# Amin-Nadimy/P-A_multigrids

Hardware: NVIDIA B200
Metric: DG DOF-updates/s per smoother sweep (higher is better)
Workload: dtype f64

## Files before the change

### p-a_multigrids_b200/csrc/pamg_api.cu

```cuda
#include <cuda_runtime.h>
#include <dlfcn.h>

#include <algorithm>
#include <cmath>
#include <cstdio>
#include <cstring>
#include <string>
#include <vector>

#include "pamg_internal.h"
#include "pamg_kernels.cuh"
#include "pamg_unstr.cuh"

using namespace pamg;

namespace {
typedef struct ncclComm* ncclComm_t;
typedef struct { char internal[128]; } ncclUniqueId;
enum { ncclUint8 = 1, ncclInt32 = 2, ncclFloat64 = 8, ncclSum = 0, ncclMax = 2, ncclMin = 3, ncclSuccess = 0 };
struct NcclApi {
  void* lib = nullptr;
  int (*GetUniqueId)(ncclUniqueId*) = nullptr;
  int (*CommInitRank)(ncclComm_t*, int, ncclUniqueId, int) = nullptr;
  int (*CommDestroy)(ncclComm_t) = nullptr;
// ... 433 lines not shown
  }
  if (g_nccl.GroupEnd() != ncclSuccess) return fail(h, PAMG_ERR_CUDA, "ncclGroupEnd failed in halo exchange");
  return PAMG_OK;
}

int launch_halo_kernel(pamg_handle* h, LevelDev& L, HaloMode mode, const double* src, double* ovl) {
  const bool cut = mode != HALO_DIRICHLET && !h->plan.peers.empty();
  if ((mode == HALO_CUT || mode == HALO_UNPACK) && !cut) return PAMG_OK;
  const int level = (int)(&L - h->lev.data()) + 1;
  HaloArgs a;
  a.tnew = src; a.told = L.told; a.ovl = ovl; a.ovl_old = L.ovl_old; a.xg = h->xg;
  a.dst_strip = h->dst_strip; a.rev = h->rev; a.strip_of = h->strip_of;
  a.bc_scale = (h->p.coarse_bc_zero && level + h->level_offset > 1) ? 0.0 : 1.0;
  a.U = h->U; a.s = L.s; a.with_old = (mode == HALO_ALL) ? 1 : 0; a.what = mode; a.nstrips = h->plan.nstrips;
  a.cut_lf = h->cut_lf; a.ncut = (int)h->plan.cut_lf.size();
  a.bc_kind = h->bc_kind; a.bc_val = h->bc_val;
  a.x.npeers = 0;
  if (cut && h->comm && h->p2p_enabled && !h->p2p_ready && !h->p2p_failed && !h->capturing && h->level_offset == 0) {
    int rc = p2p_setup(h);
    if (rc) return rc;
  }
  const bool fused_x = cut && h->p2p_ready;
  if (fused_x) { int rc = p2p_args(h, L, ovl, a.x); if (rc) return rc; }
  const long long n = (mode == HALO_CUT ? (long long)a.ncut : mode == HALO_UNPACK ? (long long)a.ncut * 3 : (long long)h->U * 3) * L.S;
  int grid = grid_for(h, n);
  if (fused_x) grid = std::min(grid, h->nsm * std::min(std::max(h->kc.halo, 1), 4));
  k_halo<<<grid, TPB, 0, h->stream>>>(a);
  h->launches++;
  CK(cudaGetLastError());
  if (cut && !fused_x) return exchange_halo_nccl(h, L, ovl);
  return PAMG_OK;
}

int exchange_told(pamg_handle* h, LevelDev& L) {
  int rc = launch_halo_kernel(h, L, HALO_CUT, L.told, L.ovl_old);
  if (!rc) halo_exchanged(L, HALO_CUT, false);
  return rc;
}

int launch_halo(pamg_handle* h, int level, HaloMode mode) {
  LevelDev& L = h->lev[level - 1];
  if (mode == HALO_UNPACK && !(h->p2p_ready && L.cut == CUT_STAGED)) return fail(h, PAMG_ERR_STATE, "nothing staged to unpack");
  int rc;
  if (mode == HALO_ALL && (rc = exchange_told(h, L))) return rc;
  if ((rc = launch_halo_kernel(h, L, mode, tnew_ptr(L), L.ovlb[L.ovl_cur]))) return rc;
  if (mode == HALO_UNPACK) unpacked(L);
  else halo_exchanged(L, mode, true);
  return PAMG_OK;
}

bool producer_level(const LevelDev& L) { return L.s >= 6 && L.s <= 8; }

int add_old_time_terms(pamg_handle* h);

int launch_build_rhs(pamg_handle* h) {
  LevelDev& L = h->lev[0];
  RhsArgs a;
  a.told = L.told; a.rhs = L.rhs; a.pc = L.pc; a.xg = h->xg; a.dt = h->p.dt; a.source_coef = h->p.source_coef;
  a.nelem = L.nelem; a.s = L.s; a.literal_source = h->p.literal_source;
  k_build_rhs<<<grid_for(h, L.nelem), TPB, 0, h->stream>>>(a);
  h->launches++;
  CK(cudaGetLastError());
  if (L.pc_old) { int rc = add_old_time_terms(h); if (rc) return rc; }
  L.rhs_valid = true;
  return PAMG_OK;
}

template <typename K>
int configure_one(pamg_handle* h, K kern, int threads, size_t smem, int& resident) {
  CK(cudaFuncSetAttribute(kern, cudaFuncAttributeMaxDynamicSharedMemorySize, (int)smem));
  CK(cudaOccupancyMaxActiveBlocksPerMultiprocessor(&resident, kern, threads, smem));
  if (resident < 1) resident = 1;
  return PAMG_OK;
}
template <bool FACE>
int configure_face(pamg_handle* h) {
  int rc, dummy = 0;
  const int f = FACE ? 1 : 0;
  if ((rc = configure_one(h, k_element_win2<MODE_JACOBI, FACE>, WIN2_THREADS, WIN_SMEM_BYTES, h->kc.win2[f]))) return rc;
  if ((rc = configure_one(h, k_element_win2<MODE_RESID, FACE>, WIN2_THREADS, WIN_SMEM_BYTES, dummy))) return rc;
  if ((rc = configure_one(h, k_element_win2<MODE_RICH, FACE>, WIN2_THREADS, WIN_SMEM_BYTES, dummy))) return rc;
  if (FACE) {
    if ((rc = configure_one(h, k_element_win2<MODE_JACOBI, FACE, true>, WIN2_THREADS, WIN_SMEM_BYTES, h->kc.win2x))) return rc;
    if ((rc = configure_one(h, k_element_win2<MODE_JACOBI, FACE, false, true>, WIN2_THREADS, WIN_SMEM_BYTES, dummy))) return rc;
    if ((rc = configure_one(h, k_element_win2<MODE_JACOBI, FACE, true, true>, WIN2_THREADS, WIN_SMEM_BYTES, dummy))) return rc;
    if ((rc = configure_one(h, k_element_win2<MODE_RICH, FACE, true>, WIN2_THREADS, WIN_SMEM_BYTES, dummy))) return rc;
  }
  if ((rc = configure_one(h, k_element_win<MODE_JACOBI, FACE>, TPB, WIN_SMEM_BYTES, h->kc.win[f]))) return rc;
  if ((rc = configure_one(h, k_element_win<MODE_RESID, FACE>, TPB, WIN_SMEM_BYTES, dummy))) return rc;
  if ((rc = configure_one(h, k_element_win<MODE_RICH, FACE>, TPB, WIN_SMEM_BYTES, dummy))) return rc;
  if (!FACE && (rc = configure_one(h, k_element_win<MODE_GS, false>, TPB, WIN_SMEM_BYTES, dummy))) return rc;
  if ((rc = configure_one(h, k_element_tma<MODE_JACOBI, FACE>, TPB, TMA_SMEM_BYTES, h->kc.tma[f]))) return rc;
  if ((rc = configure_one(h, k_element_tma<MODE_RESID, FACE>, TPB, TMA_SMEM_BYTES, dummy))) return rc;
  if ((rc = configure_one(h, k_element_tma<MODE_RICH, FACE>, TPB, TMA_SMEM_BYTES, dummy))) return rc;
  if ((rc = configure_one(h, k_element_tma<MODE_GS, FACE>, TPB, TMA_SMEM_BYTES, dummy))) return rc;
  return PAMG_OK;
}
int configure_kernels(pamg_handle* h) {
  if (h->kc.done) return PAMG_OK;
  int rc;
  if ((rc = configure_face<true>(h))) return rc;
  if ((rc = configure_face<false>(h))) return rc;
  if ((rc = configure_one(h, k_gs_win2<false>, WIN2_THREADS, GSW_SMEM_BYTES, h->kc.gs2))) return rc;
  if ((rc = configure_one(h, k_gs_win2<true>, WIN2_THREADS, GSW_SMEM_BYTES, h->kc.gs2x))) return rc;
  if ((rc = configure_one(h, k_gs_win, TPB, GSW_SMEM_BYTES, h->kc.gs))) return rc;
  CK(cudaOccupancyMaxActiveBlocksPerMultiprocessor(&h->kc.halo, k_halo, TPB, 0));
  if (h->kc.halo < 1) h->kc.halo = 1;
  cudaFuncAttributes fa;
  CK(cudaFuncGetAttributes(&fa, k_halo));
  CK(cudaFuncGetAttributes(&fa, k_gs_small));
  CK(cudaFuncGetAttributes(&fa, k_build_rhs));
  CK(cudaFuncGetAttributes(&fa, k_restrict));
  CK(cudaFuncGetAttributes(&fa, k_prolong_literal));
  CK(cudaFuncGetAttributes(&fa, k_prolong_p1));
  CK(cudaFuncGetAttributes(&fa, k_reduce_partials));
  CK(cudaFuncGetAttributes(&fa, k_fill));
  CK(cudaFuncGetAttributes(&fa, k_push));
  CK(cudaFuncGetAttributes(&fa, k_wait_flags));
  CK(cudaFuncGetAttributes(&fa, k_output_fields));
  CK(cudaFuncGetAttributes(&fa, k_element_direct2<MODE_JACOBI, true>));
  CK(cudaFuncGetAttributes(&fa, k_element_direct2<MODE_JACOBI, false>));
  CK(cudaFuncGetAttributes(&fa, k_element_direct2<MODE_RESID, true>));
  CK(cudaFuncGetAttributes(&fa, k_element_direct2<MODE_RESID, false>));
  CK(cudaFuncGetAttributes(&fa, k_element_direct2<MODE_RICH, true>));
  CK(cudaFuncGetAttributes(&fa, k_element_direct2<MODE_RICH, false>));
  CK(cudaFuncGetAttributes(&fa, k_element_direct2<MODE_GS, false>));
  h->kc.done = true;
  return PAMG_OK;
}

ElemArgs elem_args(const pamg_handle* h, const LevelDev& L, const double* Tin, double* Tout, int colour, bool use_strips,
                   bool write_next) {
  ElemArgs a;
  a.xsend = L.xsend; a.xsync = h->p2p_sync ? h->p2p_sync + (size_t)(&L - h->lev.data()) * P2P_WORDS : nullptr;
  a.Tin = Tin; a.Tout = Tout; a.rhs = L.rhs; a.ovl = L.ovlb[L.ovl_cur]; a.pc = L.pc; a.strip_of = h->strip_of; a.hmap = h->hmap;
  a.nsrc = (use_strips || Tin == Tout) ? nullptr : h->nsrc;
  a.ovl_next = write_next ? L.ovlb[L.ovl_cur ^ 1] : nullptr; a.dst_strip = h->dst_strip; a.rev = h->rev; a.nstrips = h->plan.nstrips;
  a.partial = h->partial; a.omega = h->p.omega; a.rsign = (double)h->p.residual_sign; a.nelem = L.nelem; a.s = L.s;
  a.colour = colour; a.partial_off = 0;
  return a;
}

struct ElemOverride { const double* ovl; const double* pc; double rsign; };

template <int MODE>
int launch_element(pamg_handle* h, LevelDev& L, const double* Tin, double* Tout, int colour, int grid, bool use_strips,
                   bool write_next = false, bool xchg = false, bool norm = false, const ElemOverride* ov = nullptr) {
  ElemArgs a = elem_args(h, L, Tin, Tout, colour, use_strips, write_next);
  if (MODE == MODE_RESID) xchg = false;
  if (ov) { a.ovl = ov->ovl; a.pc = ov->pc; a.rsign = ov->rsign; }
  const int f = h->p.face_terms ? 1 : 0;
  constexpr bool FACE_OK = MODE != MODE_GS;
  const bool prof = !ov && h->profiling && h->pev_used + 2 <= (int)h->pev.size();
  if (prof) CK(cudaEventRecord(h->pev[h->pev_used], h->stream));
  if (MODE != MODE_GS && producer_level(L)) {
    auto kern = xchg ? k_element_win2<MODE == MODE_RESID ? MODE_JACOBI : MODE, true, true>
                     : h->p.face_terms ? k_element_win2<MODE, true> : k_element_win2<MODE, false>;
    if (norm) kern = xchg ? k_element_win2<MODE == MODE_JACOBI ? MODE_JACOBI : MODE, true, true, MODE == MODE_JACOBI>
                          : k_element_win2<MODE == MODE_JACOBI ? MODE_JACOBI : MODE, true, false, MODE == MODE_JACOBI>;
    const int tgrid = (int)std::max(1ll, std::min(L.nelem / TPB, (long long)h->nsm * (xchg ? h->kc.win2x : h->kc.win2[f])));
    kern<<<tgrid, WIN2_THREADS, WIN_SMEM_BYTES, h->stream>>>(a);
    if (MODE == MODE_RESID || norm) h->last_partials = tgrid;
  } else if (L.C >= TPB && L.s <= 8) {
    auto kern = h->p.face_terms && FACE_OK ? k_element_win<MODE, FACE_OK> : k_element_win<MODE, false>;
    const int tgrid = (int)std::max(1ll, std::min(L.nelem / TPB, (long long)h->nsm * h->kc.win[f]));
    kern<<<tgrid, TPB, WIN_SMEM_BYTES, h->stream>>>(a);
    if (MODE == MODE_RESID) h->last_partials = tgrid;
  } else if (L.C >= TPB) {
    auto kern = h->p.face_terms ? k_element_tma<MODE, true> : k_element_tma<MODE, false>;
    const int tgrid = (int)std::max(1ll, std::min((L.nelem + TPB - 1) / TPB, (long long)h->nsm * h->kc.tma[f]));
    kern<<<tgrid, TPB, TMA_SMEM_BYTES, h->stream>>>(a);
    if (MODE == MODE_RESID) h->last_partials = tgrid;
  } else {
    if (MODE == MODE_RESID) h->last_partials = grid;
    if (h->p.face_terms && FACE_OK) k_element_direct2<MODE, FACE_OK><<<grid, TPB, 0, h->stream>>>(a);
    else k_element_direct2<MODE, false><<<grid, TPB, 0, h->stream>>>(a);
  }
  if (prof) { CK(cudaEventRecord(h->pev[h->pev_used + 1], h->stream)); h->pev_used += 2; }
  h->launches++;
  CK(cudaGetLastError());
  return PAMG_OK;
}

int add_old_time_terms(pamg_handle* h) {
  LevelDev& L = h->lev[0];
  int rc;
  if (h->p.face_terms && (rc = exchange_told(h, L))) return rc;
  const int grid = grid_for(h, L.nelem);
  if (2 * grid > h->npartial) return fail(h, PAMG_ERR_STATE, "partial buffer too small");
  const ElemOverride ov = {L.ovl_old, L.pc_old, -1.0};
  if ((rc = launch_element<MODE_RESID>(h, L, L.told, L.res, 0, grid, false, false, false, false, &ov))) return rc;
  CK(cudaMemcpyAsync(L.rhs, L.res, (size_t)L.ndof * sizeof(double), cudaMemcpyDeviceToDevice, h->stream));
  return PAMG_OK;
}

bool gs_small_ok(const pamg_handle* h, const LevelDev& L) { return h->p.face_terms && L.C <= TPB; }

int launch_gs_one_pass(pamg_handle* h, LevelDev& L, const double* Tin, double* Tout, bool use_strips, bool write_next, bool xchg) {
  const ElemArgs a = elem_args(h, L, Tin, Tout, 1, use_strips, write_next);
  if (gs_small_ok(h, L)) {
    const long long ppc = TPB / L.C, nparents = L.nelem / L.C;
    const int sgrid = (int)std::max(1ll, std::min((nparents + ppc - 1) / ppc, (long long)h->nsm * 8));
    k_gs_small<<<sgrid, TPB, 0, h->stream>>>(a);
    h->launches++;
    CK(cudaGetLastError());
    return PAMG_OK;
  }
  const bool producer = producer_level(L);
  const int resident = producer ? (xchg ? h->kc.gs2x : h->kc.gs2) : h->kc.gs;
  const bool prof = h->profiling && h->pev_used + 2 <= (int)h->pev.size();
  if (prof) CK(cudaEventRecord(h->pev[h->pev_used], h->stream));
  const int tgrid = (int)std::max(1ll, std::min(L.nelem / TPB, (long long)h->nsm * resident));
  if (producer && xchg) k_gs_win2<true><<<tgrid, WIN2_THREADS, GSW_SMEM_BYTES, h->stream>>>(a);
  else if (producer) k_gs_win2<false><<<tgrid, WIN2_THREADS, GSW_SMEM_BYTES, h->stream>>>(a);
  else k_gs_win<<<tgrid, TPB, GSW_SMEM_BYTES, h->stream>>>(a);
  if (prof) { CK(cudaEventRecord(h->pev[h->pev_used + 1], h->stream)); h->pev_used += 2; }
  h->launches++;
  CK(cudaGetLastError());
  return PAMG_OK;
}

bool norm_fusable(const pamg_handle* h, const LevelDev& L) { return h->p.face_terms && producer_level(L); }

int do_smooth(pamg_handle* h, int level, int solver, int nsweeps, bool norm_first = false) {
  LevelDev& L = h->lev[level - 1];
  if (level == 1 && !L.rhs_valid) { int rc = launch_build_rhs(h); if (rc) return rc; }
  const int grid = grid_for(h, L.nelem);
  if (solver < 1 || solver > 4) return fail(h, PAMG_ERR_ARG, "solver must be 1 (Jacobi), 2 (Richardson) or 3 (Gauss-Seidel)");
  for (int sw = 0; sw < nsweeps; ++sw) {
    L.tnew_alias = true;
    const bool gs = solver == 3 || solver == 4;
    const bool in_place = gs && !(h->p.face_terms && L.s <= 8);
    const bool fusedk = h->p.face_terms && producer_level(L);
    const bool use_strips = in_place || fusedk;
    const bool xs = fusedk && h->p2p_ready && L.xsend && !h->plan.peers.empty();
    int rc = ensure_strips(h, level, use_strips);
    if (rc) return rc;
    if (solver == 1 || solver == 2) {
      rc = (solver == 1) ? launch_element<MODE_JACOBI>(h, L, L.T[L.cur], L.T[L.cur ^ 1], 0, grid, use_strips, fusedk, xs,
                                                       norm_first && sw == 0)
                         : launch_element<MODE_RICH>(h, L, L.T[L.cur], L.T[L.cur ^ 1], 0, grid, use_strips, fusedk, xs);
      if (rc) return rc;
      L.cur ^= 1;
      L.tnew_alias = false;
    } else if (!in_place) {
      rc = launch_gs_one_pass(h, L, L.T[L.cur], L.T[L.cur ^ 1], use_strips, fusedk, xs);
      if (rc) return rc;
      L.cur ^= 1;
      L.tnew_alias = false;
    } else {
      if (sw == nsweeps - 1 && h->p.keep_tnew_gs) { rc = materialise_tnew(h, L); if (rc) return rc; }
      rc = launch_element<MODE_GS>(h, L, L.T[L.cur], L.T[L.cur], 0, grid, true);
      if (rc) return rc;
      rc = launch_element<MODE_GS>(h, L, L.T[L.cur], L.T[L.cur], 1, grid, true);
      if (rc) return rc;
    }
    if (fusedk) L.ovl_cur ^= 1;
    sweep_done(h, L, fusedk, xs);
  }
  return PAMG_OK;
}

int queue_norms(pamg_handle* h) {
  k_reduce_partials<<<1, 1024, 0, h->stream>>>(h->partial, h->last_partials, h->out3);
  h->launches++;
  CK(cudaGetLastError());
  if (h->comm && h->nranks > 1) {
    g_nccl.GroupStart();
    g_nccl.AllReduce(h->out3, h->out3, 1, ncclFloat64, ncclSum, h->comm, h->stream);
    g_nccl.AllReduce(h->out3 + 1, h->out3 + 1, 2, ncclFloat64, ncclMax, h->comm, h->stream);
    if (g_nccl.GroupEnd() != ncclSuccess) return fail(h, PAMG_ERR_CUDA, "ncclAllReduce failed");
  }
  CK(cudaMemcpyAsync(h->out3_host, h->out3, 3 * sizeof(double), cudaMemcpyDeviceToHost, h->stream));
  return PAMG_OK;
}

int do_residual(pamg_handle* h, int level, double* l2, double* linf, double* smax, bool queue_only = false) {
  LevelDev& L = h->lev[level - 1];
  if (level == 1 && !L.rhs_valid) { int rc = launch_build_rhs(h); if (rc) return rc; }
  const int grid = grid_for(h, L.nelem);
  if (2 * grid > h->npartial) return fail(h, PAMG_ERR_STATE, "partial buffer too small");
  const bool use_strips = L.strips_valid;
  int rc = ensure_strips(h, level, use_strips);
  if (rc) return rc;
  rc = launch_element<MODE_RESID>(h, L, tnew_ptr(L), L.res, 0, grid, use_strips);
  if (rc) return rc;
  if (l2 || linf || smax) {
    if ((rc = queue_norms(h))) return rc;
    if (queue_only || h->capturing) return PAMG_OK;
    CK(cudaStreamSynchronize(h->stream));
    if ((rc = p2p_check(h))) return rc;
    if (l2) *l2 = std::sqrt(h->out3_host[0]);
    if (linf) *linf = h->out3_host[1];
    if (smax) *smax = h->out3_host[2];
  }
  return PAMG_OK;
}

int do_restrict(pamg_handle* h, int fine_level) {
  if (fine_level >= (int)h->lev.size()) return PAMG_OK;
  LevelDev& F = h->lev[fine_level - 1];
  LevelDev& Cc = h->lev[fine_level];
  XferArgs a;
  a.src = F.res; a.dst = Cc.rhs; a.ncoarse = Cc.nelem; a.sc = Cc.s; a.mode = h->p.transfer;
  k_restrict<<<grid_for(h, Cc.nelem), TPB, 0, h->stream>>>(a);
  h->launches++;
  CK(cudaGetLastError());
  Cc.rhs_valid = true;
  return PAMG_OK;
}

int do_prolong(pamg_handle* h, int fine_level, bool keep_tnew = true) {
  if (fine_level >= (int)h->lev.size()) return fail(h, PAMG_ERR_ARG, "no coarser level to prolong from");
  LevelDev& F = h->lev[fine_level - 1];
  LevelDev& Cc = h->lev[fine_level];
  XferArgs a;
  a.ncoarse = Cc.nelem; a.sc = Cc.s; a.mode = h->p.transfer;
  if (h->p.transfer == 0) {
    int rc = materialise_tnew(h, F);
    if (rc) return rc;
    a.src = tnew_ptr(Cc); a.dst = F.T[F.cur ^ 1];
    k_prolong_literal<<<grid_for(h, Cc.nelem), TPB, 0, h->stream>>>(a);
  } else {
// ... 1504 lines not shown
```

### p-a_multigrids_b200/csrc/pamg_kernels.cuh

```cuda
#pragma once
#include <cstdint>

namespace pamg {

constexpr int NPC = 88;
constexpr int PC_FOLD = 24;
constexpr int PC_DPEN = 56;
constexpr int PC_WB = 60;
enum { PC_CM = 0, PC_K11 = 1, PC_K12, PC_K13, PC_K22, PC_K23, PC_K33, PC_ADV = 7, PC_FL = 10, PC_PENI = 13, PC_W = 16, PC_PENX = 19 };

constexpr int TPB = 256;

enum { MODE_JACOBI = 0, MODE_RESID = 1, MODE_GS = 2, MODE_RICH = 3 };

constexpr int P2P_SLOTS = 4;
constexpr int P2P_MAXP = 16;
enum { P2P_EPOCH = 0, P2P_COUNT = 1, P2P_WORDS = 8 };
struct P2PArgs {
  const double* send;
  int send_base;
  double* strips;
  uint4* remote[P2P_MAXP];
  long long rstride[P2P_MAXP];
  long long soff[P2P_MAXP + 1];
// ... 140 lines not shown
  const double* e = a.ovl + ((size_t)strip * S + p) * 3;
  va = __ldg(e + (hm & 3)); vb = __ldg(e + (hm >> 2));
}

__device__ __forceinline__ void halo_pair(const ElemArgs& a, int u, int mf, int slot0, int S, double& va, double& vb) {
  const int d = a.nsrc ? __ldg(a.nsrc + u * 3 + mf) : -1;
  ext_pair(a, d, __ldg(a.strip_of + u * 3 + mf), __ldg(a.hmap + u * 3 + mf), slot0, S, va, vb);
}

__device__ __forceinline__ void p2p_advance(unsigned long long* sync, unsigned long long e64) {
  if (atomicAdd(sync + P2P_COUNT, 1ull) == (unsigned long long)gridDim.x - 1) {
    sync[P2P_COUNT] = 0;
    *(volatile unsigned long long*)(sync + P2P_EPOCH) = e64 + 1;
  }
}

__device__ __forceinline__ void block_partial(double acc_sum, double acc_abs, double acc_max, double* partial) {
  for (int o = 16; o > 0; o >>= 1) {
    acc_sum += __shfl_xor_sync(0xffffffffu, acc_sum, o);
    acc_abs = fmax(acc_abs, __shfl_xor_sync(0xffffffffu, acc_abs, o));
    acc_max = fmax(acc_max, __shfl_xor_sync(0xffffffffu, acc_max, o));
  }
  __shared__ double sh[3][TPB / 32];
  const int w = threadIdx.x >> 5, l = threadIdx.x & 31;
  if (l == 0) { sh[0][w] = acc_sum; sh[1][w] = acc_abs; sh[2][w] = acc_max; }
  __syncthreads();
  if (threadIdx.x == 0) {
    double s0 = 0, s1 = 0, s2 = 0;
    for (int i = 0; i < TPB / 32; ++i) { s0 += sh[0][i]; s1 = fmax(s1, sh[1][i]); s2 = fmax(s2, sh[2][i]); }
    partial[(size_t)blockIdx.x * 3 + 0] = s0;
    partial[(size_t)blockIdx.x * 3 + 1] = s1;
    partial[(size_t)blockIdx.x * 3 + 2] = s2;
  }
}

__device__ __forceinline__ uint32_t smem_u32(const void* p) { return (uint32_t)__cvta_generic_to_shared(p); }
__device__ __forceinline__ void mbar_init(uint64_t* bar, int count) {
  asm volatile("mbarrier.init.shared::cta.b64 [%0], %1;" ::"r"(smem_u32(bar)), "r"(count) : "memory");
}
__device__ __forceinline__ void mbar_expect_tx(uint64_t* bar, uint32_t bytes) {
  asm volatile("mbarrier.arrive.expect_tx.shared::cta.b64 _, [%0], %1;" ::"r"(smem_u32(bar)), "r"(bytes) : "memory");
}
__device__ __forceinline__ void mbar_wait(uint64_t* bar, uint32_t parity) {
  asm volatile(
      "{\n"
      ".reg .pred p;\n"
      "LAB_WAIT_%=:\n"
      "mbarrier.try_wait.parity.shared::cta.b64 p, [%0], %1;\n"
      "@p bra LAB_DONE_%=;\n"
      "bra LAB_WAIT_%=;\n"
      "LAB_DONE_%=:\n"
      "}\n" ::"r"(smem_u32(bar)), "r"(parity) : "memory");
}
__device__ __forceinline__ void tma_load_1d(void* smem_dst, const void* gsrc, uint32_t bytes, uint64_t* bar) {
  asm volatile("cp.async.bulk.shared::cluster.global.mbarrier::complete_tx::bytes [%0], [%1], %2, [%3];" ::"r"(
                   smem_u32(smem_dst)), "l"(gsrc), "r"(bytes), "r"(smem_u32(bar)) : "memory");
}
__device__ __forceinline__ void tma_store_1d(void* gdst, const void* smem_src, uint32_t bytes) {
  asm volatile("cp.async.bulk.global.shared::cta.bulk_group [%0], [%1], %2;" ::"l"(gdst), "r"(smem_u32(smem_src)),
               "r"(bytes) : "memory");
}
__device__ __forceinline__ void tma_store_commit() { asm volatile("cp.async.bulk.commit_group;" ::: "memory"); }
__device__ __forceinline__ void tma_store_wait_read() { asm volatile("cp.async.bulk.wait_group.read 0;" ::: "memory"); }
__device__ __forceinline__ void tma_store_wait_all() { asm volatile("cp.async.bulk.wait_group 0;" ::: "memory"); }
__device__ __forceinline__ void fence_async_smem() { asm volatile("fence.proxy.async.shared::cta;" ::: "memory"); }

__host__ __device__ __forceinline__ void child_from_ele0(int k, int s, int& r, int& ipos, int& len) {
  const int b = 2 << s, S = 1 << s;
  int m = (int)(((float)b - sqrtf((float)(b * b - 4 * k))) * 0.5f);
  m = max(0, min(m, S - 1));
  m -= (m * (b - m) > k);
  m += (m + 1 < S) && ((m + 1) * (b - m - 1) <= k);
  m -= (m * (b - m) > k);
  r = m + 1;
  ipos = k - m * (b - m) + 1;
  len = b + 1 - 2 * r;
}

__host__ __device__ __forceinline__ void child_advance(int s, int b, int k_next, int& r, int& ipos) {
  if (k_next < TPB) { int len; child_from_ele0(k_next, s, r, ipos, len); return; }
  ipos += TPB;
  int len = b + 1 - 2 * r;
  while (ipos > len) { ipos -= len; len -= 2; ++r; }
}

constexpr int TMA_T_DOUBLES = 3 * TPB + 8;
constexpr int NSTAGE = 3;
constexpr size_t TMA_SMEM_BYTES = sizeof(double) * (NSTAGE * (TMA_T_DOUBLES + 3 * TPB) + 2 * 3 * TPB) + 16 * NSTAGE + 64;

struct ParentRegs {
  double cm, k11, k12, k13, k22, k23, k33, adv1, adv2, adv3, fl1, fl2, fl3, pi1, pi2, pi3;
  double w1, w2, w3;
  double px1, px2, px3;
};
static_assert(sizeof(ParentRegs) == 22 * sizeof(double), "ParentRegs must mirror the pc table");
__device__ __forceinline__ void load_parent(const double* __restrict__ pc, ParentRegs& P) {
  double* d = reinterpret_cast<double*>(&P);
#pragma unroll
  for (int i = 0; i < 22; ++i) d[i] = __ldg(pc + i);
}

struct Folded { double a11, a12, a13, a21, a22, a23, a31, a32, a33, c1, c2, c3, w1, w2, w3, pad; };
static_assert(sizeof(Folded) == 16 * sizeof(double), "Folded layout");

template <int MODE, bool WITH_R = false>
__device__ __forceinline__ void elem_apply_folded(const Folded& F, const double* ext, int mask, double T1, double T2,
                                                  double T3, const FaceIn& fi, double b1, double b2, double b3,
                                                  double rsign, double& o1, double& o2, double& o3, double* rr = nullptr) {
  double ax1 = F.a11 * T1 + F.a12 * T2 + F.a13 * T3;
  double ax2 = F.a21 * T1 + F.a22 * T2 + F.a23 * T3;
  double ax3 = F.a31 * T1 + F.a32 * T2 + F.a33 * T3;
  ax1 += F.c1 * (2.0 * fi.n1a + fi.n1b); ax3 += F.c1 * (fi.n1a + 2.0 * fi.n1b);
  ax3 += F.c2 * (2.0 * fi.n2a + fi.n2b); ax2 += F.c2 * (fi.n2a + 2.0 * fi.n2b);
  ax2 += F.c3 * (2.0 * fi.n3a + fi.n3b); ax1 += F.c3 * (fi.n3a + 2.0 * fi.n3b);
  double w1 = F.w1, w2 = F.w2, w3 = F.w3;
  if (mask) {
    if (mask & 1) { const double dp = ext[0], da = T1 - fi.n1a, db = T3 - fi.n1b; ax1 += dp * (2.0 * da + db); ax3 += dp * (da + 2.0 * db); }
    if (mask & 2) { const double dp = ext[1], da = T3 - fi.n2a, db = T2 - fi.n2b; ax3 += dp * (2.0 * da + db); ax2 += dp * (da + 2.0 * db); }
    if (mask & 4) { const double dp = ext[2], da = T2 - fi.n3a, db = T1 - fi.n3b; ax2 += dp * (2.0 * da + db); ax1 += dp * (da + 2.0 * db); }
    const double* wb = ext + 4 + mask * 3;
    w1 = wb[0]; w2 = wb[1]; w3 = wb[2];
  }
  if (WITH_R) { rr[0] = rsign * (ax1 - b1); rr[1] = rsign * (ax2 - b2); rr[2] = rsign * (ax3 - b3); }
  if (MODE == MODE_RESID) {
    o1 = rsign * (ax1 - b1); o2 = rsign * (ax2 - b2); o3 = rsign * (ax3 - b3);
  } else {
    o1 = T1 + w1 * (b1 - ax1); o2 = T2 + w2 * (b2 - ax2); o3 = T3 + w3 * (b3 - ax3);
  }
}

template <int MODE, bool FACE>
__device__ __forceinline__ void elem_apply_regs(const ParentRegs& P, bool up, bool interior, double T1, double T2,
                                                double T3, const FaceIn& fi, double b1, double b2, double b3,
                                                double omega, double rsign, double& o1, double& o2, double& o3) {
  const double sg = up ? 1.0 : -1.0;
  const double sumT = T1 + T2 + T3;
  const double adv = sg * sumT;
  const double mass1 = P.cm * (T1 + sumT), mass2 = P.cm * (T2 + sumT), mass3 = P.cm * (T3 + sumT);
  const double st1 = P.adv1 * adv, st2 = P.adv2 * adv, st3 = P.adv3 * adv;
  double ax1 = mass1 - st1 + (P.k11 * T1 + P.k12 * T2 + P.k13 * T3);
  double ax2 = mass2 - st2 + (P.k12 * T1 + P.k22 * T2 + P.k23 * T3);
  double ax3 = mass3 - st3 + (P.k13 * T1 + P.k23 * T2 + P.k33 * T3);
  double fx1 = 0.0, fx2 = 0.0, fx3 = 0.0;
  if (FACE) {
    {
      const double da = T1 - fi.n1a, db = T3 - fi.n1b;
      ax1 += fi.pen1 * (2.0 * da + db); ax3 += fi.pen1 * (da + 2.0 * db);
    }
    {
      const double da = T3 - fi.n2a, db = T2 - fi.n2b;
      ax3 += fi.pen2 * (2.0 * da + db); ax2 += fi.pen2 * (da + 2.0 * db);
    }
    {
      const double da = T2 - fi.n3a, db = T1 - fi.n3b;
      ax2 += fi.pen3 * (2.0 * da + db); ax1 += fi.pen3 * (da + 2.0 * db);
    }
    {
      const double fl = sg * P.fl1;
      const bool in = fl < 0.0;
      const double wa = in ? fi.n1a : T1, wb = in ? fi.n1b : T3;
      fx1 += fl * (2.0 * wa + wb); fx3 += fl * (wa + 2.0 * wb);
    }
    {
      const double fl = sg * P.fl2;
      const bool in = fl < 0.0;
      const double wa = in ? fi.n2a : T3, wb = in ? fi.n2b : T2;
// ... 299 lines not shown
        if (FACE && MODE != MODE_RICH) {
          const Folded& F = *reinterpret_cast<const Folded*>(sPC + PC_FOLD + (up ? 0 : 16));
          elem_apply_folded<MODE>(F, sPC + PC_DPEN, bmask, T1, T2, T3, fi, bb[0], bb[1], bb[2], a.rsign, o1, o2, o3);
        } else {
          elem_apply_regs<MODE, FACE>(P, up, interior, T1, T2, T3, fi, bb[0], bb[1], bb[2], a.omega, a.rsign, o1, o2, o3);
        }
      }
      bb[0] = o1; bb[1] = o2; bb[2] = o3;
      if (MODE == MODE_RESID) {
        acc_sum += o1 * o1 + o2 * o2 + o3 * o3;
        acc_abs = fmax(acc_abs, fmax(fabs(o1), fmax(fabs(o2), fabs(o3))));
        acc_max = fmax(acc_max, fmax(o1, fmax(o2, o3)));
      }
    }
    fence_async_smem();
    __syncthreads();
    if (tid == 0) {
      tma_store_1d(a.Tout + g0 * 3, sB + (it & (WIN_NB - 1)) * 3 * TPB, TILE_BYTES);
      tma_store_commit();
    }
    cur = nxt;
  }
  if (tid == 0) tma_store_wait_all();
  if (MODE == MODE_RESID) block_partial(acc_sum, acc_abs, acc_max, a.partial + (size_t)3 * a.partial_off);
}

struct StripDst { int d0, d1, d2, rv; uint4 *r0, *r1, *r2; };
__device__ __forceinline__ StripDst strip_dst_load(const ElemArgs& a, int u, int lane, unsigned long long xe = 0) {
  int d = 0, rv = 0;
  unsigned long long r = 0;
  if (lane < 3) {
    d = __ldg(a.dst_strip + u * 3 + lane); rv = __ldg(a.rev + u * 3 + lane) << lane;
    if (xe != 0) {
      const ulonglong2 t = __ldg(a.xsend + u * 3 + lane);
      if (t.x) r = t.x + (xe & (P2P_SLOTS - 1)) * t.y * sizeof(uint4);
    }
  }
  StripDst o;
  o.d0 = __shfl_sync(0xffffffffu, d, 0); o.d1 = __shfl_sync(0xffffffffu, d, 1); o.d2 = __shfl_sync(0xffffffffu, d, 2);
  o.rv = __shfl_sync(0xffffffffu, rv, 0) | __shfl_sync(0xffffffffu, rv, 1) | __shfl_sync(0xffffffffu, rv, 2);
  o.r0 = (uint4*)__shfl_sync(0xffffffffu, r, 0); o.r1 = (uint4*)__shfl_sync(0xffffffffu, r, 1); o.r2 = (uint4*)__shfl_sync(0xffffffffu, r, 2);
  return o;
}

__device__ __forceinline__ void strips_from_tile(const ElemArgs& a, const double* __restrict__ tile, const StripDst& sd, int k0,
                                                 int s, int& m0, int lane, unsigned long long xe = 0) {
  const int S = 1 << s, b = 2 << s;
  const int kend = k0 + TPB;
  auto put = [&](int dst, uint4* rbase, int rvf, int pos, int k) {
    const int slot = rvf ? (S - 1 - pos) : pos;
    const double* t = tile + (k - k0) * 3;
    if (rbase != nullptr) {
      const unsigned e = (unsigned)xe;
#pragma unroll
      for (int i = 0; i < 3; ++i) {
        const unsigned long long v = (unsigned long long)__double_as_longlong(t[i]);
        asm volatile("st.volatile.global.v4.u32 [%0], {%1, %2, %3, %4};" ::"l"(rbase + slot * 3 + i), "r"((unsigned)v), "r"(e), "r"((unsigned)(v >> 32)), "r"(e) : "memory");
      }
      return;
    }
    double* e = a.ovl_next + ((size_t)dst * S + slot) * 3;
    e[0] = t[0]; e[1] = t[1]; e[2] = t[2];
  };
  if (sd.d0 >= 0 && k0 < b - 1) {
    const int e1 = min(kend, b - 1);
    for (int k = k0 + 2 * lane; k < e1; k += 64) put(sd.d0, sd.r0, sd.rv & 1, k >> 1, k);
  }
  while ((m0 + 1) * (b - m0 - 1) <= k0) ++m0;
  if (sd.d1 >= 0 || sd.d2 >= 0) {
    for (int m = m0 + lane; m < S; m += 32) {
      const int first = m * (b - m);
      if (first >= kend) break;
      const int last = (m + 1) * (b - m - 1) - 1;
      if (sd.d2 >= 0 && first >= k0) put(sd.d2, sd.r2, sd.rv & 4, m, first);
      if (sd.d1 >= 0 && last < kend) put(sd.d1, sd.r1, sd.rv & 2, m, last);
    }
  }
}

constexpr int WIN2_THREADS = TPB + 32;
__device__ __forceinline__ void named_arrive(int id, int count) { asm volatile("bar.arrive %0, %1;" ::"r"(id), "r"(count) : "memory"); }
__device__ __forceinline__ void named_sync(int id, int count) { asm volatile("bar.sync %0, %1;" ::"r"(id), "r"(count) : "memory"); }

template <int MODE, bool FACE, bool XCHG = false, bool NORM = false>
__global__ void __launch_bounds__(WIN2_THREADS, 3) k_element_win2(ElemArgs a) {
  extern __shared__ __align__(128) unsigned char dsm[];
  double* sT = reinterpret_cast<double*>(dsm);
  double* sB = sT + 3 * WIN_CH;
  uint64_t* barT = reinterpret_cast<uint64_t*>(sB + 3 * TPB * WIN_NB);
  uint64_t* barB = barT + WIN_NT;
  __shared__ __align__(16) double sPC2[2][NPC];
  __shared__ int sIdx2[2][12];
  __shared__ double shp[3][TPB / 32];
  const int s = a.s, twos = 2 * s, b = 2 << s, S = 1 << s;
  const long long Cmask = (1ll << twos) - 1;
  const int tid = threadIdx.x;
  constexpr uint32_t TILE_BYTES = 3 * TPB * sizeof(double);
  double acc_sum = 0.0, acc_abs = 0.0, acc_max = 0.0;
  if (tid == 0) {
    for (int i = 0; i < WIN_NT + WIN_NB; ++i) mbar_init(&barT[i], 1);
    asm volatile("fence.mbarrier_init.release.cluster;" ::: "memory");
  }
  __syncthreads();
  const long long ntiles = a.nelem / TPB;
  const long long per = (ntiles + gridDim.x - 1) / gridDim.x;
  const long long tbeg = (long long)blockIdx.x * per, tend = min(ntiles, tbeg + per);
  const long long tlo = max(0ll, tbeg - 2), thi = min(ntiles, tend + 2);

  if (tid >= TPB) {
    const int lane = tid - TPB;
    int u_loaded = -1;
    unsigned long long e64 = 0;
    if (XCHG) e64 = *(volatile unsigned long long*)(a.xsync + P2P_EPOCH);
    auto issueT = [&](long long tile) {
      const int sl = (int)(tile & (WIN_NT - 1));
      mbar_expect_tx(&barT[sl], TILE_BYTES);
      tma_load_1d(sT + sl * 3 * TPB, a.Tin + tile * 3 * TPB, TILE_BYTES, &barT[sl]);
    };
    auto issueB = [&](long long tile) {
      const int u = (int)((tile * TPB) >> twos);
      if (u != u_loaded) {
        for (int i = lane; i < NPC; i += 32) sPC2[u & 1][i] = __ldg(a.pc + (size_t)u * NPC + i);
        if (lane < 3) {
          sIdx2[u & 1][lane] = __ldg(a.strip_of + u * 3 + lane); sIdx2[u & 1][4 + lane] = __ldg(a.hmap + u * 3 + lane);
          sIdx2[u & 1][8 + lane] = a.nsrc ? __ldg(a.nsrc + u * 3 + lane) : -1;
        }
        u_loaded = u;
        __syncwarp();
      }
      if (lane == 0) {
        const int sl = (int)((tile - tbeg) & (WIN_NB - 1));
        mbar_expect_tx(&barB[sl], TILE_BYTES);
        tma_load_1d(sB + sl * 3 * TPB, a.rhs + tile * 3 * TPB, TILE_BYTES, &barB[sl]);
      }
    };
    if (tbeg < tend) {
      if (lane == 0) for (long long t = tlo; t < min(thi, tbeg + 6); ++t) issueT(t);
      for (long long t = tbeg; t < min(tend, tbeg + 3); ++t) issueB(t);
    }
    int m0 = 0, u_m0 = -1;
    StripDst sd = {-1, -1, -1, 0, nullptr, nullptr, nullptr};
    for (long long p = tbeg; p < tend; ++p) {
      const int it = (int)(p - tbeg);
      named_sync(1 + (it & 3), WIN2_THREADS);
      if (lane == 0) {
        tma_store_1d(a.Tout + p * 3 * TPB, sB + (it & (WIN_NB - 1)) * 3 * TPB, TILE_BYTES);
        tma_store_commit();
        if (p + 6 < thi) issueT(p + 6);
        if (p + 3 < tend) tma_store_wait_read1();
      }
      __syncwarp();
      if (p + 3 < tend) issueB(p + 3);
      if (MODE != MODE_RESID && a.ovl_next) {
        const int u = (int)((p * TPB) >> twos);
        if (u != u_m0) { m0 = 0; u_m0 = u; sd = strip_dst_load(a, u, lane, XCHG ? e64 + 1 : 0); }
        strips_from_tile(a, sB + (it & (WIN_NB - 1)) * 3 * TPB, sd, (int)((p * TPB) & Cmask), s, m0, lane, XCHG ? e64 + 1 : 0);
      }
    }
    if (XCHG && MODE != MODE_RESID && lane == 0) p2p_advance(a.xsync, e64);
    if (lane == 0) tma_store_wait_all();
  } else {
    const int tbegi = (int)tbeg, tendi = (int)tend, tloi = (int)tlo, thii = (int)thi;
    const int pshift = twos - 8;
    const unsigned kmask = (unsigned)Cmask;
    struct Prep { int r, ipos, len; double h1a, h1b, h2a, h2b; };
    auto prepare = [&](int tile, int u_cur, bool first, Prep& p) {
      p.h1a = 0.0; p.h1b = 0.0; p.h2a = 0.0; p.h2b = 0.0;
      if (tile >= tendi) return;
      const int kk = (int)((((unsigned)tile << 8) + (unsigned)tid) & kmask);
      if (first) child_from_ele0(kk, s, p.r, p.ipos, p.len);
      else child_advance(s, b, kk, p.r, p.ipos);
      p.len = b + 1 - 2 * p.r;
      if (!FACE || !(p.ipos & 1)) return;
      const bool f1 = p.r == 1, side = p.ipos == 1 || p.ipos == p.len;
      if (f1 | side) {
        const int u = tile >> pshift;
        const bool same = u == u_cur;
        const int* ix = sIdx2[u & 1];
        if (f1) {
          const int strip = same ? ix[0] : __ldg(a.strip_of + u * 3), hm = same ? ix[4] : __ldg(a.hmap + u * 3);
          const int d = same ? ix[8] : (a.nsrc ? __ldg(a.nsrc + u * 3) : -1);
          ext_pair(a, d, strip, hm, p.ipos >> 1, S, p.h1a, p.h1b);
        }
        if (side) {
          const int mf = (p.ipos == 1) ? 2 : 1;
          const int strip = same ? ix[mf] : __ldg(a.strip_of + u * 3 + mf), hm = same ? ix[4 + mf] : __ldg(a.hmap + u * 3 + mf);
          const int d = same ? ix[8 + mf] : (a.nsrc ? __ldg(a.nsrc + u * 3 + mf) : -1);
          ext_pair(a, d, strip, hm, p.r - 1, S, p.h2a, p.h2b);
        }
      }
    };
    Prep cur, nxt;
    cur.r = 2; cur.ipos = 2; cur.len = 3;
    prepare(tbegi, -1, true, cur);
    for (int tile = tbegi; tile < tendi; ++tile) {
      const int it = tile - tbegi;
      const int u_tile = tile >> pshift;
      if (it == 0) {
        for (int tw = tloi; tw <= min(tile + 2, thii - 1); ++tw) mbar_wait(&barT[tw & (WIN_NT - 1)], (uint32_t)(((tw - tloi) >> 3) & 1));
      } else if (tile + 2 < thii) {
        mbar_wait(&barT[(tile + 2) & (WIN_NT - 1)], (uint32_t)(((tile + 2 - tloi) >> 3) & 1));
      }
      mbar_wait(&barB[it & (WIN_NB - 1)], (uint32_t)((it / WIN_NB) & 1));
      nxt.r = cur.r; nxt.ipos = cur.ipos;
      prepare(tile + 1, u_tile, false, nxt);
      const double* sPC = sPC2[u_tile & 1];
      double* bb = sB + (it & (WIN_NB - 1)) * (3 * TPB) + tid * 3;
      {
        const int cw = ((tile & (WIN_NT - 1)) << 8) + tid;
        const double* t = sT + cw * 3;
        const double T1 = t[0], T2 = t[1], T3 = t[2];
        const bool up = cur.ipos & 1;
        double o1, o2, o3;
        FaceIn fi;
        int bmask = 0;
        bool interior = true;
        const ParentRegs& P = *reinterpret_cast<const ParentRegs*>(sPC);
        if (FACE) {
          fi.pen1 = P.pi1; fi.pen2 = P.pi2; fi.pen3 = P.pi3;
          const int dv = up ? (2 * cur.r - b - 2) : (b - 2 * cur.r);
          const double* tv = sT + ((cw + dv) & (WIN_CH - 1)) * 3;
          fi.n1a = tv[2]; fi.n1b = tv[0];
          const double* tl = sT + ((cw - 1) & (WIN_CH - 1)) * 3;
          const double* tr = sT + ((cw + 1) & (WIN_CH - 1)) * 3;
          const double* t2 = up ? tl : tr;
          const double* t3 = up ? tr : tl;
          fi.n2a = t2[1]; fi.n2b = t2[2];
          fi.n3a = t3[0]; fi.n3b = t3[1];
          if (up && (cur.r == 1 || cur.ipos == 1 || cur.ipos == cur.len)) {
            interior = false;
            if (cur.r == 1) { fi.n1a = cur.h1a; fi.n1b = cur.h1b; fi.pen1 = P.px1; bmask |= 1; }
            if (cur.ipos == 1) { fi.n2a = cur.h2a; fi.n2b = cur.h2b; fi.pen2 = P.px2; bmask |= 2; }
            if (cur.ipos == cur.len) {
              if (cur.len == 1) halo_pair(a, u_tile, 1, cur.r - 1, S, fi.n3a, fi.n3b);
              else { fi.n3a = cur.h2a; fi.n3b = cur.h2b; }
              fi.pen3 = P.px3; bmask |= 4;
            }
          }
        }
        if (FACE && MODE != MODE_RICH) {
          const Folded& F = *reinterpret_cast<const Folded*>(sPC + PC_FOLD + (up ? 0 : 16));
          if (NORM) {
            double rr[3];
            elem_apply_folded<MODE, true>(F, sPC + PC_DPEN, bmask, T1, T2, T3, fi, bb[0], bb[1], bb[2], a.rsign, o1, o2, o3, rr);
            acc_sum += rr[0] * rr[0] + rr[1] * rr[1] + rr[2] * rr[2];
            acc_abs = fmax(acc_abs, fmax(fabs(rr[0]), fmax(fabs(rr[1]), fabs(rr[2]))));
            acc_max = fmax(acc_max, fmax(rr[0], fmax(rr[1], rr[2])));
          } else {
            elem_apply_folded<MODE>(F, sPC + PC_DPEN, bmask, T1, T2, T3, fi, bb[0], bb[1], bb[2], a.rsign, o1, o2, o3);
          }
        } else {
          elem_apply_regs<MODE, FACE>(P, up, interior, T1, T2, T3, fi, bb[0], bb[1], bb[2], a.omega, a.rsign, o1, o2, o3);
        }
        bb[0] = o1; bb[1] = o2; bb[2] = o3;
        if (MODE == MODE_RESID) {
          acc_sum += o1 * o1 + o2 * o2 + o3 * o3;
          acc_abs = fmax(acc_abs, fmax(fabs(o1), fmax(fabs(o2), fabs(o3))));
          acc_max = fmax(acc_max, fmax(o1, fmax(o2, o3)));
        }
      }
      fence_async_smem();
      named_arrive(1 + (it & 3), WIN2_THREADS);
      cur = nxt;
    }
  }
  if (MODE == MODE_RESID || NORM) {
    if (tid < TPB) {
      for (int o = 16; o > 0; o >>= 1) {
        acc_sum += __shfl_xor_sync(0xffffffffu, acc_sum, o);
        acc_abs = fmax(acc_abs, __shfl_xor_sync(0xffffffffu, acc_abs, o));
        acc_max = fmax(acc_max, __shfl_xor_sync(0xffffffffu, acc_max, o));
      }
      if ((tid & 31) == 0) { shp[0][tid >> 5] = acc_sum; shp[1][tid >> 5] = acc_abs; shp[2][tid >> 5] = acc_max; }
    }
    __syncthreads();
    if (tid == 0) {
      double s0 = 0, s1 = 0, s2 = 0;
      for (int i = 0; i < TPB / 32; ++i) { s0 += shp[0][i]; s1 = fmax(s1, shp[1][i]); s2 = fmax(s2, shp[2][i]); }
      double* partial = a.partial + (size_t)3 * a.partial_off;
      partial[(size_t)blockIdx.x * 3 + 0] = s0; partial[(size_t)blockIdx.x * 3 + 1] = s1; partial[(size_t)blockIdx.x * 3 + 2] = s2;
    }
  }
}

constexpr size_t GSW_SMEM_BYTES = WIN_SMEM_BYTES;
__device__ __forceinline__ void tma_store_wait_read2() { asm volatile("cp.async.bulk.wait_group.read 2;" ::: "memory"); }

__global__ void __launch_bounds__(TPB, 3) k_gs_win(ElemArgs a) {
  extern __shared__ __align__(128) unsigned char dsm[];
  double* sT = reinterpret_cast<double*>(dsm);
  double* sB = sT + 3 * WIN_CH;
  uint64_t* barT = reinterpret_cast<uint64_t*>(sB + 3 * TPB * WIN_NB);
// ... 881 lines not shown
```

Baseline: 251.9 billion.

## Alternate Jacobi sweep tile traversal direction to reuse L2-resident data

Adds a REV template variant of the windowed element kernel that walks tiles in reverse physical order, and uses it on odd Jacobi sweeps. Each block's tile range, TMA loads and stores, child index stepping (new child_retreat) and strip extraction are remapped so that consecutive sweeps alternate direction. The intent is that the tail of the previous sweep's output is still in L2 when the next sweep starts reading it. The cost is extra index arithmetic and a backward strip-cursor adjustment. Ring-buffer slot mapping and the order of neighbour halos now depend on reversed indexing, which carries correctness risk.

```diff
diff --git a/p-a_multigrids_b200/csrc/pamg_api.cu b/p-a_multigrids_b200/csrc/pamg_api.cu
--- a/p-a_multigrids_b200/csrc/pamg_api.cu
+++ b/p-a_multigrids_b200/csrc/pamg_api.cu
@@ -539,6 +539,7 @@
   if ((rc = configure_one(h, k_element_win2<MODE_RICH, FACE>, WIN2_THREADS, WIN_SMEM_BYTES, dummy))) return rc;
   if (FACE) {
     if ((rc = configure_one(h, k_element_win2<MODE_JACOBI, FACE, true>, WIN2_THREADS, WIN_SMEM_BYTES, h->kc.win2x))) return rc;
+    if ((rc = configure_one(h, k_element_win2<MODE_JACOBI, true, false, false, true>, WIN2_THREADS, WIN_SMEM_BYTES, dummy))) return rc;
     if ((rc = configure_one(h, k_element_win2<MODE_JACOBI, FACE, false, true>, WIN2_THREADS, WIN_SMEM_BYTES, dummy))) return rc;
     if ((rc = configure_one(h, k_element_win2<MODE_JACOBI, FACE, true, true>, WIN2_THREADS, WIN_SMEM_BYTES, dummy))) return rc;
     if ((rc = configure_one(h, k_element_win2<MODE_RICH, FACE, true>, WIN2_THREADS, WIN_SMEM_BYTES, dummy))) return rc;
@@ -602,7 +603,8 @@
 
 template <int MODE>
 int launch_element(pamg_handle* h, LevelDev& L, const double* Tin, double* Tout, int colour, int grid, bool use_strips,
-                   bool write_next = false, bool xchg = false, bool norm = false, const ElemOverride* ov = nullptr) {
+                   bool write_next = false, bool xchg = false, bool norm = false, const ElemOverride* ov = nullptr,
+                   bool rev = false) {
   ElemArgs a = elem_args(h, L, Tin, Tout, colour, use_strips, write_next);
   if (MODE == MODE_RESID) xchg = false;
   if (ov) { a.ovl = ov->ovl; a.pc = ov->pc; a.rsign = ov->rsign; }
@@ -615,6 +617,7 @@
                      : h->p.face_terms ? k_element_win2<MODE, true> : k_element_win2<MODE, false>;
     if (norm) kern = xchg ? k_element_win2<MODE == MODE_JACOBI ? MODE_JACOBI : MODE, true, true, MODE == MODE_JACOBI>
                           : k_element_win2<MODE == MODE_JACOBI ? MODE_JACOBI : MODE, true, false, MODE == MODE_JACOBI>;
+    else if (rev && MODE == MODE_JACOBI && h->p.face_terms && !xchg) kern = k_element_win2<MODE, true, false, false, MODE == MODE_JACOBI>;
     const int tgrid = (int)std::max(1ll, std::min(L.nelem / TPB, (long long)h->nsm * (xchg ? h->kc.win2x : h->kc.win2[f])));
     kern<<<tgrid, WIN2_THREADS, WIN_SMEM_BYTES, h->stream>>>(a);
     if (MODE == MODE_RESID || norm) h->last_partials = tgrid;
@@ -695,7 +698,7 @@
     if (rc) return rc;
     if (solver == 1 || solver == 2) {
       rc = (solver == 1) ? launch_element<MODE_JACOBI>(h, L, L.T[L.cur], L.T[L.cur ^ 1], 0, grid, use_strips, fusedk, xs,
-                                                       norm_first && sw == 0)
+                                                       norm_first && sw == 0, nullptr, (sw & 1) != 0)
                          : launch_element<MODE_RICH>(h, L, L.T[L.cur], L.T[L.cur ^ 1], 0, grid, use_strips, fusedk, xs);
       if (rc) return rc;
       L.cur ^= 1;
diff --git a/p-a_multigrids_b200/csrc/pamg_kernels.cuh b/p-a_multigrids_b200/csrc/pamg_kernels.cuh
--- a/p-a_multigrids_b200/csrc/pamg_kernels.cuh
+++ b/p-a_multigrids_b200/csrc/pamg_kernels.cuh
@@ -246,6 +246,12 @@
   ipos += TPB;
   int len = b + 1 - 2 * r;
   while (ipos > len) { ipos -= len; len -= 2; ++r; }
+}
+
+__host__ __device__ __forceinline__ void child_retreat(int s, int b, int k_next, int& r, int& ipos) {
+  if (k_next + TPB >= (1 << (2 * s))) { int len; child_from_ele0(k_next, s, r, ipos, len); return; }
+  ipos -= TPB;
+  while (ipos < 1) { --r; ipos += b + 1 - 2 * r; }
 }
 
 constexpr int TMA_T_DOUBLES = 3 * TPB + 8;
@@ -711,8 +717,9 @@
 __device__ __forceinline__ void named_arrive(int id, int count) { asm volatile("bar.arrive %0, %1;" ::"r"(id), "r"(count) : "memory"); }
 __device__ __forceinline__ void named_sync(int id, int count) { asm volatile("bar.sync %0, %1;" ::"r"(id), "r"(count) : "memory"); }
 
-template <int MODE, bool FACE, bool XCHG = false, bool NORM = false>
+template <int MODE, bool FACE, bool XCHG = false, bool NORM = false, bool REV = false>
 __global__ void __launch_bounds__(WIN2_THREADS, 3) k_element_win2(ElemArgs a) {
+  static_assert(!REV || (!NORM && MODE != MODE_RESID), "partial norms are summed in forward tile order");
   extern __shared__ __align__(128) unsigned char dsm[];
   double* sT = reinterpret_cast<double*>(dsm);
   double* sB = sT + 3 * WIN_CH;
@@ -733,8 +740,10 @@
   __syncthreads();
   const long long ntiles = a.nelem / TPB;
   const long long per = (ntiles + gridDim.x - 1) / gridDim.x;
-  const long long tbeg = (long long)blockIdx.x * per, tend = min(ntiles, tbeg + per);
+  const long long pbeg = (long long)blockIdx.x * per, pend = min(ntiles, pbeg + per);
+  const long long tbeg = REV ? ntiles - pend : pbeg, tend = REV ? ntiles - pbeg : pend;
   const long long tlo = max(0ll, tbeg - 2), thi = min(ntiles, tend + 2);
+  auto phys = [&](long long q) { return REV ? ntiles - 1 - q : q; };
 
   if (tid >= TPB) {
     const int lane = tid - TPB;
@@ -742,12 +751,13 @@
     unsigned long long e64 = 0;
     if (XCHG) e64 = *(volatile unsigned long long*)(a.xsync + P2P_EPOCH);
     auto issueT = [&](long long tile) {
-      const int sl = (int)(tile & (WIN_NT - 1));
+      const long long pt = phys(tile);
+      const int sl = (int)(pt & (WIN_NT - 1));
       mbar_expect_tx(&barT[sl], TILE_BYTES);
-      tma_load_1d(sT + sl * 3 * TPB, a.Tin + tile * 3 * TPB, TILE_BYTES, &barT[sl]);
+      tma_load_1d(sT + sl * 3 * TPB, a.Tin + pt * 3 * TPB, TILE_BYTES, &barT[sl]);
     };
     auto issueB = [&](long long tile) {
-      const int u = (int)((tile * TPB) >> twos);
+      const int u = (int)((phys(tile) * TPB) >> twos);
       if (u != u_loaded) {
         for (int i = lane; i < NPC; i += 32) sPC2[u & 1][i] = __ldg(a.pc + (size_t)u * NPC + i);
         if (lane < 3) {
@@ -760,7 +770,7 @@
       if (lane == 0) {
         const int sl = (int)((tile - tbeg) & (WIN_NB - 1));
         mbar_expect_tx(&barB[sl], TILE_BYTES);
-        tma_load_1d(sB + sl * 3 * TPB, a.rhs + tile * 3 * TPB, TILE_BYTES, &barB[sl]);
+        tma_load_1d(sB + sl * 3 * TPB, a.rhs + phys(tile) * 3 * TPB, TILE_BYTES, &barB[sl]);
       }
     };
     if (tbeg < tend) {
@@ -773,7 +783,7 @@
       const int it = (int)(p - tbeg);
       named_sync(1 + (it & 3), WIN2_THREADS);
       if (lane == 0) {
-        tma_store_1d(a.Tout + p * 3 * TPB, sB + (it & (WIN_NB - 1)) * 3 * TPB, TILE_BYTES);
+        tma_store_1d(a.Tout + phys(p) * 3 * TPB, sB + (it & (WIN_NB - 1)) * 3 * TPB, TILE_BYTES);
         tma_store_commit();
         if (p + 6 < thi) issueT(p + 6);
         if (p + 3 < tend) tma_store_wait_read1();
@@ -781,9 +791,11 @@
       __syncwarp();
       if (p + 3 < tend) issueB(p + 3);
       if (MODE != MODE_RESID && a.ovl_next) {
-        const int u = (int)((p * TPB) >> twos);
+        const int u = (int)((phys(p) * TPB) >> twos);
+        const int k0 = (int)((phys(p) * TPB) & Cmask);
         if (u != u_m0) { m0 = 0; u_m0 = u; sd = strip_dst_load(a, u, lane, XCHG ? e64 + 1 : 0); }
-        strips_from_tile(a, sB + (it & (WIN_NB - 1)) * 3 * TPB, sd, (int)((p * TPB) & Cmask), s, m0, lane, XCHG ? e64 + 1 : 0);
+        if (REV) while (m0 > 0 && m0 * (b - m0) > k0) --m0;
+        strips_from_tile(a, sB + (it & (WIN_NB - 1)) * 3 * TPB, sd, k0, s, m0, lane, XCHG ? e64 + 1 : 0);
       }
     }
     if (XCHG && MODE != MODE_RESID && lane == 0) p2p_advance(a.xsync, e64);
@@ -792,18 +804,21 @@
     const int tbegi = (int)tbeg, tendi = (int)tend, tloi = (int)tlo, thii = (int)thi;
     const int pshift = twos - 8;
     const unsigned kmask = (unsigned)Cmask;
+    const int nt1 = (int)ntiles - 1;
+    auto physi = [&](int q) { return REV ? nt1 - q : q; };
     struct Prep { int r, ipos, len; double h1a, h1b, h2a, h2b; };
     auto prepare = [&](int tile, int u_cur, bool first, Prep& p) {
       p.h1a = 0.0; p.h1b = 0.0; p.h2a = 0.0; p.h2b = 0.0;
       if (tile >= tendi) return;
-      const int kk = (int)((((unsigned)tile << 8) + (unsigned)tid) & kmask);
+      const int kk = (int)((((unsigned)physi(tile) << 8) + (unsigned)tid) & kmask);
       if (first) child_from_ele0(kk, s, p.r, p.ipos, p.len);
+      else if (REV) child_retreat(s, b, kk, p.r, p.ipos);
       else child_advance(s, b, kk, p.r, p.ipos);
       p.len = b + 1 - 2 * p.r;
       if (!FACE || !(p.ipos & 1)) return;
       const bool f1 = p.r == 1, side = p.ipos == 1 || p.ipos == p.len;
       if (f1 | side) {
-        const int u = tile >> pshift;
+        const int u = physi(tile) >> pshift;
         const bool same = u == u_cur;
         const int* ix = sIdx2[u & 1];
         if (f1) {
@@ -824,11 +839,11 @@
     prepare(tbegi, -1, true, cur);
     for (int tile = tbegi; tile < tendi; ++tile) {
       const int it = tile - tbegi;
-      const int u_tile = tile >> pshift;
+      const int u_tile = physi(tile) >> pshift;
       if (it == 0) {
-        for (int tw = tloi; tw <= min(tile + 2, thii - 1); ++tw) mbar_wait(&barT[tw & (WIN_NT - 1)], (uint32_t)(((tw - tloi) >> 3) & 1));
+        for (int tw = tloi; tw <= min(tile + 2, thii - 1); ++tw) mbar_wait(&barT[physi(tw) & (WIN_NT - 1)], (uint32_t)(((tw - tloi) >> 3) & 1));
       } else if (tile + 2 < thii) {
-        mbar_wait(&barT[(tile + 2) & (WIN_NT - 1)], (uint32_t)(((tile + 2 - tloi) >> 3) & 1));
+        mbar_wait(&barT[physi(tile + 2) & (WIN_NT - 1)], (uint32_t)(((tile + 2 - tloi) >> 3) & 1));
       }
       mbar_wait(&barB[it & (WIN_NB - 1)], (uint32_t)((it / WIN_NB) & 1));
       nxt.r = cur.r; nxt.ipos = cur.ipos;
@@ -836,7 +851,7 @@
       const double* sPC = sPC2[u_tile & 1];
       double* bb = sB + (it & (WIN_NB - 1)) * (3 * TPB) + tid * 3;
       {
-        const int cw = ((tile & (WIN_NT - 1)) << 8) + tid;
+        const int cw = ((physi(tile) & (WIN_NT - 1)) << 8) + tid;
         const double* t = sT + cw * 3;
         const double T1 = t[0], T2 = t[1], T3 = t[2];
         const bool up = cur.ipos & 1;
```

Result: no change. 250.8 billion (median of 6 runs) (-0.4%).
